# Ecogenomics/CheckM

Hardware: NVIDIA H100
Metric: genomes/hour (higher is better)
Workload: dtype int16 (SSV) / u8 (MSV) / int16 (Viterbi) / f32 (Forward, domain definition)

## Files before the change

checkm_b200/csrc/fwdback_blk.cuh:

```cuda
#pragma once
#include "device_utils.cuh"
#include "engine.hpp"
#include "fwdback.cuh"

namespace ckm {

constexpr int BLK_LOOKAHEAD_MAXQ = 16;

template <int Q, bool TSMEM>
struct BlkModel {
  int M;
  const float *rfb;
  const float4 *tsm;
  float4 t0[TSMEM ? 1 : Q], t1[TSMEM ? 1 : Q];
  int lane;
  __device__ __forceinline__ float4 T0(int q) const { return TSMEM ? tsm[q * 32 + lane] : t0[TSMEM ? 0 : q]; }
  __device__ __forceinline__ float4 T1(int q) const { return TSMEM ? tsm[(Q + q) * 32 + lane] : t1[TSMEM ? 0 : q]; }
};

template <int Q, bool TSMEM>
__device__ __forceinline__ void blk_model_load(BlkModel<Q, TSMEM> &bm, const ModelScalars &ms, const float4 *tfb, const float *rfb,
                                               float4 *tsm, int lane) {
  bm.M = ms.M; bm.lane = lane;
  bm.rfb = rfb + ms.blk_off * 32 * KPAD + lane;
  bm.tsm = tsm;
  const float4 *src = tfb + ms.blk_off * 32 * 2;
  if (TSMEM) {
    __syncwarp();
    for (int q = 0; q < Q; ++q) { tsm[q * 32 + lane] = __ldg(src + (q * 32 + lane) * 2); tsm[(Q + q) * 32 + lane] = __ldg(src + (q * 32 + lane) * 2 + 1); }
    __syncwarp();
  } else {
#pragma unroll
    for (int q = 0; q < Q; ++q) { bm.t0[TSMEM ? 0 : q] = __ldg(src + (q * 32 + lane) * 2); bm.t1[TSMEM ? 0 : q] = __ldg(src + (q * 32 + lane) * 2 + 1); }
  }
}

template <int Q, bool TSMEM, bool FULL, bool STORE_D = true>
__device__ __forceinline__ float forward_blk(const BlkModel<Q, TSMEM> &bm, const uint8_t *__restrict__ res, int L, const Specials sp,
                                             float *xmx, float *full) {
  const int lane = bm.lane;
  float Mx[Q], Ix[Q], Dx[Q];
#pragma unroll
  for (int q = 0; q < Q; ++q) { Mx[q] = 0.0f; Ix[q] = 0.0f; Dx[q] = 0.0f; }
  if (FULL) {
#pragma unroll
    for (int z = 0; z < 3 * Q; ++z) full[z * 32 + lane] = 0.0f;
  }
  float xE = 0.0f, xN = 1.0f, xJ = 0.0f, xB = sp.nmove, xC = 0.0f, totscale = 0.0f;
  if (xmx != nullptr && lane == 0) { xmx[X_E] = xE; xmx[X_N] = xN; xmx[X_J] = xJ; xmx[X_B] = xB; xmx[X_C] = xC; xmx[X_SCALE] = 1.0f; }
  constexpr bool LA = (Q <= BLK_LOOKAHEAD_MAXQ);
  float ecur[Q];
  int xnext;
  if (LA) {
    const float *rp = bm.rfb + (size_t)((L >= 1) ? __ldg(res) : 0) * Q * 32;
#pragma unroll
    for (int q = 0; q < Q; ++q) ecur[q] = __ldg(rp + q * 32);
    xnext = (L >= 2) ? __ldg(res + 1) : 0;
  } else xnext = (L >= 1) ? __ldg(res) : 0;
  for (int i = 1; i <= L; ++i) {
    float enext[LA ? Q : 1];
    {
      const float *rp = bm.rfb + (size_t)xnext * Q * 32;
      if (LA) {
#pragma unroll
        for (int q = 0; q < Q; ++q) enext[LA ? q : 0] = __ldg(rp + q * 32);
        xnext = (i + 2 <= L) ? __ldg(res + i + 1) : 0;
      } else {
#pragma unroll
        for (int q = 0; q < Q; ++q) ecur[q] = __ldg(rp + q * 32);
        xnext = (i + 1 <= L) ? __ldg(res + i) : 0;
      }
    }
    float pm_in = __shfl_up_sync(0xffffffffu, Mx[Q - 1], 1), pi_in = __shfl_up_sync(0xffffffffu, Ix[Q - 1], 1), pd_in = __shfl_up_sync(0xffffffffu, Dx[Q - 1], 1);
    if (lane == 0) { pm_in = 0.0f; pi_in = 0.0f; pd_in = 0.0f; }
    float md[Q], esum = 0.0f;
#pragma unroll
    for (int q = Q - 1; q >= 0; --q) {
      const float4 t0 = bm.T0(q), t1 = bm.T1(q);
      const float pm = (q > 0) ? Mx[q - 1] : pm_in, pi = (q > 0) ? Ix[q - 1] : pi_in, pd = (q > 0) ? Dx[q - 1] : pd_in;
      float sv = xB * t0.x;
      sv += pm * t0.y;
      sv += pi * t0.z;
      sv += pd * t0.w;
      sv *= ecur[q];
      const float nI = Mx[q] * t1.y + Ix[q] * t1.z;
      md[q] = sv * t1.x;
      Mx[q] = sv; Ix[q] = nI;
      esum += sv;
    }
    float Bb = 0.0f, Tb = 1.0f;
#pragma unroll
    for (int q = 0; q < Q; ++q) { const float tdd = bm.T1(q).w; Bb = md[q] + Bb * tdd; Tb *= tdd; }
    float Bs = Bb, Ts = Tb;
#pragma unroll
    for (int o = 1; o < 32; o <<= 1) {
      const float Bl = __shfl_up_sync(0xffffffffu, Bs, o), Tl = __shfl_up_sync(0xffffffffu, Ts, o);
      if (lane >= o) { Bs = Bs + Bl * Ts; Ts = Ts * Tl; }
    }
    float d = __shfl_up_sync(0xffffffffu, Bs, 1);
    if (lane == 0) d = 0.0f;
#pragma unroll
    for (int q = 0; q < Q; ++q) {
      const bool in = (lane * Q + q + 1) <= bm.M;
      Dx[q] = in ? d : 0.0f;
      esum += Dx[q];
      d = md[q] + d * bm.T1(q).w;
    }
    xE = warp_sum_float(esum);
    xN = xN * sp.nloop;
    xC = (xC * sp.nloop) + (xE * sp.emove);
    xJ = (xJ * sp.nloop) + (xE * sp.eloop);
    xB = (xJ * sp.nmove) + (xN * sp.nmove);
    float scale = 1.0f;
    if (xE > 1.0e4f) {
      scale = xE;
      const float inv = __fdiv_rn(1.0f, xE);
      xN = __fdiv_rn(xN, xE); xC = __fdiv_rn(xC, xE); xJ = __fdiv_rn(xJ, xE); xB = __fdiv_rn(xB, xE);
#pragma unroll
      for (int q = 0; q < Q; ++q) { Mx[q] *= inv; Dx[q] *= inv; Ix[q] *= inv; }
      totscale += (float)log((double)xE);
      xE = 1.0f;
    }
    if (FULL) {
      float *fr = full + (size_t)i * 3 * Q * 32 + lane;
#pragma unroll
      for (int q = 0; q < Q; ++q) { fr[q * 32] = Mx[q]; if (STORE_D) fr[(Q + q) * 32] = Dx[q]; fr[(2 * Q + q) * 32] = Ix[q]; }
    }
    if (xmx != nullptr && lane == 0) {
      float *xr = xmx + (size_t)i * X_NX;
      xr[X_E] = xE; xr[X_N] = xN; xr[X_J] = xJ; xr[X_B] = xB; xr[X_C] = xC; xr[X_SCALE] = scale;
    }
    if (LA) {
#pragma unroll
      for (int q = 0; q < Q; ++q) ecur[q] = enext[LA ? q : 0];
    }
  }
  return totscale + (float)log((double)(xC * sp.nmove));
}

__device__ __forceinline__ void prefetch_l2(const void *p) { asm volatile("prefetch.global.L2 [%0];" ::"l"(p)); }
template <int Q, bool TSMEM, int MODE>
__device__ __forceinline__ void backward_blk(const BlkModel<Q, TSMEM> &bm, const uint8_t *__restrict__ res, int L, const Specials sp,
                                             const float *fxmx, float *bxmx, float *full) {
  const int lane = bm.lane, M = bm.M;
  float Mx[Q], Ix[Q], Dx[Q];
#pragma unroll
  for (int q = 0; q < Q; ++q) { Mx[q] = 0.0f; Ix[q] = 0.0f; Dx[q] = 0.0f; }
  float xC = 0.0f, xE = 0.0f, xJ = 0.0f, xN = 0.0f, xB = 0.0f;
  constexpr bool LA = (Q <= BLK_LOOKAHEAD_MAXQ);
  float ecur[Q];
#pragma unroll
  for (int q = 0; q < Q; ++q) ecur[q] = 0.0f;
  int xnext = (L >= 1) ? __ldg(res + L - 1) : 0;
  for (int i = L; i >= 0; --i) {
    float enext[LA ? Q : 1];
    if (LA) {
      const float *rp = bm.rfb + (size_t)xnext * Q * 32;
#pragma unroll
      for (int q = 0; q < Q; ++q) enext[LA ? q : 0] = __ldg(rp + q * 32);
      xnext = (i >= 2) ? __ldg(res + i - 2) : 0;
    } else if (i < L) {
      const float *rp = bm.rfb + (size_t)xnext * Q * 32;
#pragma unroll
      for (int q = 0; q < Q; ++q) ecur[q] = __ldg(rp + q * 32);
      xnext = (i >= 1) ? __ldg(res + i - 1) : 0;
    }
    if (MODE == 2 && i >= 3) {
      const float *fr = full + (size_t)(i - 2) * 3 * Q * 32;
      if (lane < Q) { prefetch_l2(fr + lane * 32); prefetch_l2(fr + (2 * Q + lane) * 32); }
    }
    float em[Q];
    if (i == L) {
      xC = sp.nmove; xE = xC * sp.emove; xB = 0.0f; xJ = 0.0f; xN = 0.0f;
#pragma unroll
      for (int q = 0; q < Q; ++q) em[q] = 0.0f;
    } else {
      float part = 0.0f;
#pragma unroll
      for (int q = 0; q < Q; ++q) { em[q] = Mx[q] * ecur[q]; part += em[q] * bm.T0(q).x; }
      xB = warp_sum_float(part);
      xC = xC * sp.nloop;
      xJ = (xB * sp.nmove) + (xJ * sp.nloop);
      xN = (xB * sp.nmove) + (xN * sp.nloop);
      xE = (xC * sp.emove) + (xJ * sp.eloop);
    }
    const float s = (i >= 1) ? fxmx[(size_t)i * X_NX + X_SCALE] : 1.0f;
    if (i >= 1) {
      const float inv = (s > 1.0f) ? __fdiv_rn(1.0f, s) : 1.0f;
      float em_next = __shfl_down_sync(0xffffffffu, em[0], 1);
      float4 tn_next;
      {
        const float4 mine = bm.T0(0);
        tn_next.x = 0.0f;
        tn_next.y = __shfl_down_sync(0xffffffffu, mine.y, 1); tn_next.z = __shfl_down_sync(0xffffffffu, mine.z, 1); tn_next.w = __shfl_down_sync(0xffffffffu, mine.w, 1);
      }
      if (lane == 31) { em_next = 0.0f; tn_next.y = 0.0f; tn_next.z = 0.0f; tn_next.w = 0.0f; }
      float cb[Q];
      float Bb = 0.0f, Tb = 1.0f;
#pragma unroll
      for (int q = Q - 1; q >= 0; --q) {
        const int k = lane * Q + q + 1;
        const float mnext = (q < Q - 1) ? em[q + 1] : em_next;
        const float tdm = (q < Q - 1) ? bm.T0(q + 1).w : tn_next.w;
        const bool in = (k <= M);
        cb[q] = in ? (xE + ((k < M) ? mnext * tdm : 0.0f)) : 0.0f;
        const float tdd = in ? bm.T1(q).w : 0.0f;
        Bb = cb[q] + Bb * tdd; Tb *= tdd;
      }
      float Bs = Bb, Ts = Tb;
#pragma unroll
      for (int o = 1; o < 32; o <<= 1) {
        const float Br = __shfl_down_sync(0xffffffffu, Bs, o), Tr = __shfl_down_sync(0xffffffffu, Ts, o);
        if (lane + o < 32) { Bs = Bs + Br * Ts; Ts = Ts * Tr; }
      }
      float dnext = __shfl_down_sync(0xffffffffu, Bs, 1);
      if (lane == 31) dnext = 0.0f;
      float nM[Q], nI[Q], nD[Q];
#pragma unroll
      for (int q = Q - 1; q >= 0; --q) {
        const int k = lane * Q + q + 1;
        const bool in = (k <= M);
        const float4 t1 = bm.T1(q);
        const float mnext = (q < Q - 1) ? em[q + 1] : em_next;
        const float4 tn = (q < Q - 1) ? bm.T0(q + 1) : tn_next;
        const float tmm = (k < M) ? tn.y : 0.0f, tim = (k < M) ? tn.z : 0.0f;
        const float inext = (i < L) ? Ix[q] : 0.0f;
        const float dv = in ? (cb[q] + dnext * t1.w) : 0.0f;
        float mv = xE + mnext * tmm + inext * t1.y + dnext * t1.x;
        float iv = mnext * tim + inext * t1.z;
        if (!in) { mv = 0.0f; iv = 0.0f; }
        nM[q] = mv * inv; nI[q] = iv * inv; nD[q] = dv * inv;
        dnext = dv;
      }
#pragma unroll
      for (int q = 0; q < Q; ++q) { Mx[q] = nM[q]; Ix[q] = nI[q]; Dx[q] = nD[q]; }
      if (s > 1.0f) { xE = __fdiv_rn(xE, s); xN = __fdiv_rn(xN, s); xJ = __fdiv_rn(xJ, s); xB = __fdiv_rn(xB, s); xC = __fdiv_rn(xC, s); }
    } else {
      xC = 0.0f; xJ = 0.0f; xE = 0.0f;
#pragma unroll
      for (int q = 0; q < Q; ++q) { Mx[q] = 0.0f; Ix[q] = 0.0f; Dx[q] = 0.0f; }
    }
    if (MODE == 1) {
      float *fr = full + (size_t)i * 3 * Q * 32 + lane;
#pragma unroll
      for (int q = 0; q < Q; ++q) { fr[q * 32] = Mx[q]; fr[(Q + q) * 32] = Dx[q]; fr[(2 * Q + q) * 32] = Ix[q]; }
    }
    if (MODE == 2 && i >= 1) {
      float *fr = full + (size_t)i * 3 * Q * 32 + lane;
      float fm[Q], fi[Q];
#pragma unroll
      for (int q = 0; q < Q; ++q) { fm[q] = fr[q * 32]; fi[q] = fr[(2 * Q + q) * 32]; }
#pragma unroll
      for (int q = 0; q < Q; ++q) { fr[q * 32] = fm[q] * Mx[q]; fr[(2 * Q + q) * 32] = fi[q] * Ix[q]; }
    }
    if (bxmx != nullptr && lane == 0) {
      float *xr = bxmx + (size_t)i * X_NX;
      xr[X_E] = xE; xr[X_N] = xN; xr[X_J] = xJ; xr[X_B] = xB; xr[X_C] = xC; xr[X_SCALE] = s;
    }
    if (LA) {
#pragma unroll
      for (int q = 0; q < Q; ++q) ecur[q] = enext[LA ? q : 0];
    }
  }
}

}
```

checkm_b200/csrc/kernels_blk.cu:

```cuda
#include "engine.hpp"
#include "device_utils.cuh"
#include "stages.hpp"
#include "fwdback.cuh"
#include "fwdback_blk.cuh"
#include "domdef_common.cuh"
#include "filter_common.cuh"

namespace ckm {

constexpr int BLK_WARPS = 4;

__host__ __device__ constexpr size_t blk_tsm_bytes(int Q) { return (size_t)Q * 32 * 2 * sizeof(float4); }

template <int Q, bool TSMEM>
__global__ void __launch_bounds__(BLK_WARPS * 32) fwd2_kernel(FilterParams p) {
  extern __shared__ __align__(16) uint8_t bsm[];
  const int lane = threadIdx.x & 31, warp = threadIdx.x >> 5;
  float4 *tsm = reinterpret_cast<float4 *>(bsm) + (size_t)warp * Q * 32 * 2;
  const int n = min(*p.in_count, p.in_cap);
  for (int c = blockIdx.x * BLK_WARPS + warp; c < n; c += gridDim.x * BLK_WARPS) {
    Candidate cd = p.in[c];
    const ModelScalars ms = p.ms[cd.model];
    if (ms.vq != Q) continue;
    const int s = cd.seq, L = p.len[s];
    BlkModel<Q, TSMEM> bm;
    blk_model_load<Q, TSMEM>(bm, ms, p.tfb, p.rfb, tsm, lane);
    const float fsc = forward_blk<Q, TSMEM, false>(bm, p.res + p.off[s], L, make_specials(L, true), nullptr, nullptr);
    fwd_verdict(p, cd, fsc, ms, lane);
  }
}

template <int Q, bool TSMEM>
__global__ void __launch_bounds__(BLK_WARPS * 32) regions2_kernel(DomdefParams p) {
  extern __shared__ __align__(16) uint8_t bsm[];
  const int lane = threadIdx.x & 31, warp = threadIdx.x >> 5;
  float4 *tsm = reinterpret_cast<float4 *>(bsm) + (size_t)warp * Q * 32 * 2;
  for (int idx = p.pair_begin + blockIdx.x * BLK_WARPS + warp; idx < p.pair_end; idx += gridDim.x * BLK_WARPS) {
    const int pi = p.pair_order[idx];
    const PairWork pw = p.pairs[pi];
    const ModelScalars ms = p.ms[pw.model];
    if (ms.vq != Q) continue;
    const int L = pw.L;
    BlkModel<Q, TSMEM> bm;
    blk_model_load<Q, TSMEM>(bm, ms, p.tfb, p.rfb, tsm, lane);
    const uint8_t *res = p.res + p.off[pw.seq];
    const Specials sp = make_specials(L, true);
    float *xf = p.xf + pw.row_off * X_NX, *xb = p.xb + pw.row_off * X_NX;
    forward_blk<Q, TSMEM, false>(bm, res, L, sp, xf, nullptr);
    __syncwarp();
    backward_blk<Q, TSMEM, 0>(bm, res, L, sp, xf, xb, nullptr);
    __syncwarp();
    regions_tail(p, pi, L, sp, xf, xb, p.btot + pw.row_off, p.etot + pw.row_off, p.mocc + pw.row_off, p.n2sc + pw.row_off, lane);
    __syncwarp();
  }
}

template <int Q> struct BlockedLayout {
  const float *F; const float4 *tfb; int M;
  static __device__ __forceinline__ int at(int k) { return ((k - 1) % Q) * 32 + (k - 1) / Q; }
  __device__ __forceinline__ float cell(int row, int plane, int k) const { return F[((int64_t)row * 3 + plane) * (Q * 32) + at(k)]; }
  __device__ __forceinline__ float4 t0(int k) const { return __ldg(tfb + at(k) * 2); }
  __device__ __forceinline__ float4 t1(int k) const { return __ldg(tfb + at(k) * 2 + 1); }
  __device__ __forceinline__ void row_best(int row, int lane, float &bm, int &bk, float &bd, int &bdk) const {
    const float *dpc = F + (int64_t)row * 3 * (Q * 32) + lane;
    if constexpr (Q <= 12) {
#pragma unroll
      for (int q = 0; q < Q; ++q) {
        const int kk = lane * Q + q + 1;
        if (kk <= M) {
          const float v = dpc[q * 32]; if (v >= bm) { bm = v; bk = kk; }
          const float w = dpc[(Q + q) * 32]; if (w > bd) { bd = w; bdk = kk; }
        }
      }
    } else {
#pragma unroll 4
      for (int q = 0; q < Q; ++q) {
        const int kk = lane * Q + q + 1;
        if (kk <= M) { const float v = dpc[q * 32]; if (v >= bm) { bm = v; bk = kk; } }
      }
#pragma unroll 4
      for (int q = 0; q < Q; ++q) {
        const int kk = lane * Q + q + 1;
        if (kk <= M) { const float w = dpc[(Q + q) * 32]; if (w > bd) { bd = w; bdk = kk; } }
      }
    }
  }
};

template <int Q, bool TSMEM>
__global__ void __launch_bounds__(BLK_WARPS * 32) envelope2_kernel(DomdefParams p) {
  extern __shared__ __align__(16) uint8_t bsm[];
  const int lane = threadIdx.x & 31, warp = threadIdx.x >> 5;
  float4 *tsm = reinterpret_cast<float4 *>(bsm) + (size_t)warp * Q * 32 * 2;
  float *null2 = reinterpret_cast<float *>(bsm + (TSMEM ? BLK_WARPS * blk_tsm_bytes(Q) : 0)) + warp * 32;
  constexpr int QW = Q * 32;
  for (int idx = p.env_begin + blockIdx.x * BLK_WARPS + warp; idx < p.env_end; idx += gridDim.x * BLK_WARPS) {
    const int ei = p.env_order[idx];
    const Envelope env = p.envs[ei];
    const PairWork pw = p.pairs[env.pair];
    const ModelScalars ms = p.ms[pw.model];
    if (ms.vq != Q) continue;
    BlkModel<Q, TSMEM> bm;
    blk_model_load<Q, TSMEM>(bm, ms, p.tfb, p.rfb, tsm, lane);
    const int M = ms.M, Ld = env.j - env.i + 1;
    const uint8_t *res = p.res + p.off[pw.seq] + (env.i - 1);
    const Specials sp = make_specials(pw.L, false);
    const int64_t mat = (int64_t)(Ld + 1) * 3 * QW;
    float *F = p.scratch + env.scratch_off, *Bm = F;
    float *xf = F + mat, *xb = xf + (int64_t)(Ld + 1) * X_NX, *pps = xb + (int64_t)(Ld + 1) * X_NX;
    float *xo = xf;
    float *n2sc = p.n2sc + pw.row_off;
    const float envsc = forward_blk<Q, TSMEM, true, false>(bm, res, Ld, sp, xf, F);
    __syncwarp();
    backward_blk<Q, TSMEM, 2>(bm, res, Ld, sp, xf, xb, F);
    __syncwarp();
    const float scaleproduct = __fdiv_rn(1.0f, xb[X_N]);
    float em[Q], ein[Q];
#pragma unroll
    for (int q = 0; q < Q; ++q) { em[q] = 0.0f; ein[q] = 0.0f; }
    for (int r = 1; r <= Ld; ++r) {
      if (r + 2 <= Ld && lane < Q) {
        const float *fn = F + (int64_t)(r + 2) * 3 * QW;
        prefetch_l2(fn + lane * 32); prefetch_l2(fn + (2 * Q + lane) * 32);
      }
      const float totr = scaleproduct * xf[(int64_t)r * X_NX + X_SCALE];
      const float *fr = F + (int64_t)r * 3 * QW + lane;
      float vm[Q], vi[Q];
#pragma unroll
      for (int q = 0; q < Q; ++q) { vm[q] = fr[q * 32]; vi[q] = fr[(2 * Q + q) * 32]; }
#pragma unroll
      for (int q = 0; q < Q; ++q) {
        const float pm = vm[q] * totr, pi = vi[q] * totr;
        em[q] = (r == 1) ? pm : em[q] + pm;
        ein[q] = (r == 1) ? pi : ein[q] + pi;
      }
    }
    special_posteriors(sp, xf, xb, scaleproduct, pps, Ld, lane);
    const bool range_err = isinf(scaleproduct);
    if (!range_err && !env.null2_done) {
      const float norm = __fdiv_rn(1.0f, (float)Ld);
      const float xfactor = special_xfactor(pps, Ld, norm, lane);
#pragma unroll
      for (int q = 0; q < Q; ++q) { em[q] *= norm; ein[q] *= norm; }
      for (int x = 0; x < K; ++x) {
        const float *rp = bm.rfb + (size_t)x * QW;
        float part = 0.0f;
#pragma unroll
        for (int q = 0; q < Q; ++q) { part += em[q] * __ldg(rp + q * 32); part += ein[q]; }
        part = warp_sum_float(part);
        if (lane == 0) null2[x] = part + xfactor;
      }
      null2_finish(null2, n2sc, res, env, lane);
    }
    float oasc = 0.0f;
    const float NINF = -INFINITY;
    if (!range_err) {
      float oM[Q], oI[Q], oD[Q];
#pragma unroll
      for (int q = 0; q < Q; ++q) { oM[q] = NINF; oI[q] = NINF; oD[q] = NINF; }
#pragma unroll
      for (int z = 0; z < 3 * Q; ++z) Bm[z * 32 + lane] = NINF;
      OaSpecials os(sp);
      os.store(xo, lane);
      for (int r = 1; r <= Ld; ++r) {
        if (r + 2 <= Ld && lane < Q) {
          const float *fn = F + (int64_t)(r + 2) * 3 * QW;
          prefetch_l2(fn + lane * 32); prefetch_l2(fn + (2 * Q + lane) * 32);
        }
        const float totr = scaleproduct * xf[(int64_t)r * X_NX + X_SCALE];
        const float *ppr = F + (int64_t)r * 3 * QW + lane;
        float *orow = Bm + (int64_t)r * 3 * QW + lane;
        float ppm[Q], ppi[Q];
#pragma unroll
        for (int q = 0; q < Q; ++q) { ppm[q] = ppr[q * 32]; ppi[q] = ppr[(2 * Q + q) * 32]; }
        float pm_in = __shfl_up_sync(0xffffffffu, oM[Q - 1], 1), pi_in = __shfl_up_sync(0xffffffffu, oI[Q - 1], 1), pd_in = __shfl_up_sync(0xffffffffu, oD[Q - 1], 1);
        if (lane == 0) { pm_in = NINF; pi_in = NINF; pd_in = NINF; }
        float a[Q]; bool ps[Q];
        float emax = NINF;
#pragma unroll
        for (int q = Q - 1; q >= 0; --q) {
          const float4 t0 = bm.T0(q), t1 = bm.T1(q);
          const bool in = (lane * Q + q + 1) <= M;
          const float pm = (q > 0) ? oM[q - 1] : pm_in, pi = (q > 0) ? oI[q - 1] : pi_in, pd = (q > 0) ? oD[q - 1] : pd_in;
          float sv = (t0.x > 0.0f) ? os.B : 0.0f;
          sv = fmaxf(sv, (t0.y > 0.0f) ? pm : 0.0f);
          sv = fmaxf(sv, (t0.z > 0.0f) ? pi : 0.0f);
          sv = fmaxf(sv, (t0.w > 0.0f) ? pd : 0.0f);
          sv += ppm[q] * totr;
          if (!in) sv = NINF;
          const float nI = in ? fmaxf((t1.y > 0.0f) ? oM[q] : 0.0f, (t1.z > 0.0f) ? oI[q] : 0.0f) + ppi[q] * totr : NINF;
          a[q] = (t1.x > 0.0f) ? sv : 0.0f;
          ps[q] = (t1.w > 0.0f);
          if (!in) { a[q] = NINF; ps[q] = true; }
          if (!ps[q]) a[q] = fmaxf(a[q], 0.0f);
          oM[q] = sv; oI[q] = nI;
          emax = fmaxf(emax, sv);
        }
        float A = NINF; bool pass = true;
#pragma unroll
        for (int q = 0; q < Q; ++q) { if (ps[q]) { A = fmaxf(a[q], A); } else { A = a[q]; pass = false; } }
        float As = A; bool Ps = pass;
#pragma unroll
        for (int o = 1; o < 32; o <<= 1) {
          const float Al = __shfl_up_sync(0xffffffffu, As, o);
          const int pl = __shfl_up_sync(0xffffffffu, (int)Ps, o);
          if (lane >= o && Ps) { As = fmaxf(As, Al); Ps = (pl != 0); }
        }
        float d = __shfl_up_sync(0xffffffffu, As, 1);
        if (lane == 0) d = NINF;
#pragma unroll
        for (int q = 0; q < Q; ++q) {
          const bool in = (lane * Q + q + 1) <= M;
          oD[q] = in ? d : NINF;
          emax = fmaxf(emax, oD[q]);
          d = ps[q] ? fmaxf(a[q], d) : a[q];
        }
#pragma unroll
        for (int o = 16; o > 0; o >>= 1) emax = fmaxf(emax, __shfl_xor_sync(0xffffffffu, emax, o));
        os.row(sp, pps + r * 3, emax);
#pragma unroll
        for (int q = 0; q < Q; ++q) { orow[q * 32] = oM[q]; orow[(Q + q) * 32] = oD[q]; orow[(2 * Q + q) * 32] = oI[q]; }
        os.store(xo + (int64_t)r * X_NX, lane);
      }
      oasc = os.C;
    }
    __syncwarp();
    OaTrace tr;
    if (!range_err) tr = oa_traceback(BlockedLayout<Q>{Bm, p.tfb + ms.blk_off * 64, M}, p, pw, env, sp, xo, pps, Ld, M, lane);
    write_domain(p, env, n2sc, tr, envsc, oasc, lane);
    __syncwarp();
  }
}

template <class P, class KF>
static int launch_blk(KF kern, const char *name, int Q, bool tsmem, const P &p, int grid, size_t extra, cudaStream_t st) {
  return launch_kernel(kern, name, grid, BLK_WARPS * 32, (tsmem ? BLK_WARPS * blk_tsm_bytes(Q) : 0) + extra, st, p);
}
int launch_fwd2(const FilterParams &p, int cls, int grid, cudaStream_t st) {
  return with_class(cls, [&](auto Q, auto TSMEM) { return launch_blk(fwd2_kernel<Q, TSMEM>, "fwd2_kernel", Q, TSMEM, p, grid, 0, st); });
}
int launch_regions2(const DomdefParams &p, int cls, int grid, cudaStream_t st) {
  return with_class(cls, [&](auto Q, auto TSMEM) { return launch_blk(regions2_kernel<Q, TSMEM>, "regions2_kernel", Q, TSMEM, p, grid, 0, st); });
}
int launch_envelopes2(const DomdefParams &p, int cls, int grid, cudaStream_t st) {
  return with_class(cls, [&](auto Q, auto TSMEM) {
    return launch_blk(envelope2_kernel<Q, TSMEM>, "envelope2_kernel", Q, TSMEM, p, grid, BLK_WARPS * 32 * sizeof(float), st);
  });
}

}
```

Before: 35540.

## Recompute forward rows in envelope OA pass instead of storing full matrix

For small Q the envelope kernel no longer stores the full forward DP matrix. Backward writes its M/I rows, and the optimal-accuracy pass recomputes each forward row on the fly to form posteriors. The null2 posterior sums are folded into that same pass, with the accumulators kept in shared memory for some Q, and launch bounds gain minimum-block hints. This trades extra forward arithmetic for much less global-memory traffic to the scratch matrix, but it risks register pressure and occupancy changes.

```diff
diff --git a/checkm_b200/csrc/fwdback_blk.cuh b/checkm_b200/csrc/fwdback_blk.cuh
--- a/checkm_b200/csrc/fwdback_blk.cuh
+++ b/checkm_b200/csrc/fwdback_blk.cuh
@@ -35,29 +35,26 @@
   }
 }
 
-template <int Q, bool TSMEM, bool FULL, bool STORE_D = true>
-__device__ __forceinline__ float forward_blk(const BlkModel<Q, TSMEM> &bm, const uint8_t *__restrict__ res, int L, const Specials sp,
-                                             float *xmx, float *full) {
-  const int lane = bm.lane;
+template <int Q, bool TSMEM>
+struct FwdRows {
+  static constexpr bool LA = (Q <= BLK_LOOKAHEAD_MAXQ);
   float Mx[Q], Ix[Q], Dx[Q];
-#pragma unroll
-  for (int q = 0; q < Q; ++q) { Mx[q] = 0.0f; Ix[q] = 0.0f; Dx[q] = 0.0f; }
-  if (FULL) {
-#pragma unroll
-    for (int z = 0; z < 3 * Q; ++z) full[z * 32 + lane] = 0.0f;
-  }
-  float xE = 0.0f, xN = 1.0f, xJ = 0.0f, xB = sp.nmove, xC = 0.0f, totscale = 0.0f;
-  if (xmx != nullptr && lane == 0) { xmx[X_E] = xE; xmx[X_N] = xN; xmx[X_J] = xJ; xmx[X_B] = xB; xmx[X_C] = xC; xmx[X_SCALE] = 1.0f; }
-  constexpr bool LA = (Q <= BLK_LOOKAHEAD_MAXQ);
+  float xE, xN, xJ, xB, xC, totscale;
   float ecur[Q];
   int xnext;
-  if (LA) {
-    const float *rp = bm.rfb + (size_t)((L >= 1) ? __ldg(res) : 0) * Q * 32;
-#pragma unroll
-    for (int q = 0; q < Q; ++q) ecur[q] = __ldg(rp + q * 32);
-    xnext = (L >= 2) ? __ldg(res + 1) : 0;
-  } else xnext = (L >= 1) ? __ldg(res) : 0;
-  for (int i = 1; i <= L; ++i) {
+  __device__ __forceinline__ void init(const BlkModel<Q, TSMEM> &bm, const uint8_t *__restrict__ res, int L, const Specials &sp) {
+#pragma unroll
+    for (int q = 0; q < Q; ++q) { Mx[q] = 0.0f; Ix[q] = 0.0f; Dx[q] = 0.0f; }
+    xE = 0.0f; xN = 1.0f; xJ = 0.0f; xB = sp.nmove; xC = 0.0f; totscale = 0.0f;
+    if (LA) {
+      const float *rp = bm.rfb + (size_t)((L >= 1) ? __ldg(res) : 0) * Q * 32;
+#pragma unroll
+      for (int q = 0; q < Q; ++q) ecur[q] = __ldg(rp + q * 32);
+      xnext = (L >= 2) ? __ldg(res + 1) : 0;
+    } else xnext = (L >= 1) ? __ldg(res) : 0;
+  }
+  __device__ __forceinline__ float row(const BlkModel<Q, TSMEM> &bm, const uint8_t *__restrict__ res, int L, const Specials &sp, int i) {
+    const int lane = bm.lane;
     float enext[LA ? Q : 1];
     {
       const float *rp = bm.rfb + (size_t)xnext * Q * 32;
@@ -121,21 +118,39 @@
       totscale += (float)log((double)xE);
       xE = 1.0f;
     }
+    if (LA) {
+#pragma unroll
+      for (int q = 0; q < Q; ++q) ecur[q] = enext[LA ? q : 0];
+    }
+    return scale;
+  }
+  __device__ __forceinline__ float score(const Specials &sp) const { return totscale + (float)log((double)(xC * sp.nmove)); }
+};
+
+template <int Q, bool TSMEM, bool FULL = false, bool STORE_D = true>
+__device__ __forceinline__ float forward_blk(const BlkModel<Q, TSMEM> &bm, const uint8_t *__restrict__ res, int L, const Specials sp,
+                                             float *xmx, float *full = nullptr) {
+  const int lane = bm.lane;
+  FwdRows<Q, TSMEM> f;
+  f.init(bm, res, L, sp);
+  if (FULL) {
+#pragma unroll
+    for (int z = 0; z < 3 * Q; ++z) full[z * 32 + lane] = 0.0f;
+  }
+  if (xmx != nullptr && lane == 0) { xmx[X_E] = f.xE; xmx[X_N] = f.xN; xmx[X_J] = f.xJ; xmx[X_B] = f.xB; xmx[X_C] = f.xC; xmx[X_SCALE] = 1.0f; }
+  for (int i = 1; i <= L; ++i) {
+    const float scale = f.row(bm, res, L, sp, i);
     if (FULL) {
       float *fr = full + (size_t)i * 3 * Q * 32 + lane;
 #pragma unroll
-      for (int q = 0; q < Q; ++q) { fr[q * 32] = Mx[q]; if (STORE_D) fr[(Q + q) * 32] = Dx[q]; fr[(2 * Q + q) * 32] = Ix[q]; }
+      for (int q = 0; q < Q; ++q) { fr[q * 32] = f.Mx[q]; if (STORE_D) fr[(Q + q) * 32] = f.Dx[q]; fr[(2 * Q + q) * 32] = f.Ix[q]; }
     }
     if (xmx != nullptr && lane == 0) {
       float *xr = xmx + (size_t)i * X_NX;
-      xr[X_E] = xE; xr[X_N] = xN; xr[X_J] = xJ; xr[X_B] = xB; xr[X_C] = xC; xr[X_SCALE] = scale;
-    }
-    if (LA) {
-#pragma unroll
-      for (int q = 0; q < Q; ++q) ecur[q] = enext[LA ? q : 0];
-    }
-  }
-  return totscale + (float)log((double)(xC * sp.nmove));
+      xr[X_E] = f.xE; xr[X_N] = f.xN; xr[X_J] = f.xJ; xr[X_B] = f.xB; xr[X_C] = f.xC; xr[X_SCALE] = scale;
+    }
+  }
+  return f.score(sp);
 }
 
 __device__ __forceinline__ void prefetch_l2(const void *p) { asm volatile("prefetch.global.L2 [%0];" ::"l"(p)); }
@@ -240,10 +255,10 @@
 #pragma unroll
       for (int q = 0; q < Q; ++q) { Mx[q] = 0.0f; Ix[q] = 0.0f; Dx[q] = 0.0f; }
     }
-    if (MODE == 1) {
+    if (MODE == 1 && i >= 1) {
       float *fr = full + (size_t)i * 3 * Q * 32 + lane;
 #pragma unroll
-      for (int q = 0; q < Q; ++q) { fr[q * 32] = Mx[q]; fr[(Q + q) * 32] = Dx[q]; fr[(2 * Q + q) * 32] = Ix[q]; }
+      for (int q = 0; q < Q; ++q) { fr[q * 32] = Mx[q]; fr[(2 * Q + q) * 32] = Ix[q]; }
     }
     if (MODE == 2 && i >= 1) {
       float *fr = full + (size_t)i * 3 * Q * 32 + lane;
diff --git a/checkm_b200/csrc/kernels_blk.cu b/checkm_b200/csrc/kernels_blk.cu
--- a/checkm_b200/csrc/kernels_blk.cu
+++ b/checkm_b200/csrc/kernels_blk.cu
@@ -25,7 +25,7 @@
     const int s = cd.seq, L = p.len[s];
     BlkModel<Q, TSMEM> bm;
     blk_model_load<Q, TSMEM>(bm, ms, p.tfb, p.rfb, tsm, lane);
-    const float fsc = forward_blk<Q, TSMEM, false>(bm, p.res + p.off[s], L, make_specials(L, true), nullptr, nullptr);
+    const float fsc = forward_blk<Q, TSMEM>(bm, p.res + p.off[s], L, make_specials(L, true), nullptr);
     fwd_verdict(p, cd, fsc, ms, lane);
   }
 }
@@ -46,7 +46,7 @@
     const uint8_t *res = p.res + p.off[pw.seq];
     const Specials sp = make_specials(L, true);
     float *xf = p.xf + pw.row_off * X_NX, *xb = p.xb + pw.row_off * X_NX;
-    forward_blk<Q, TSMEM, false>(bm, res, L, sp, xf, nullptr);
+    forward_blk<Q, TSMEM>(bm, res, L, sp, xf);
     __syncwarp();
     backward_blk<Q, TSMEM, 0>(bm, res, L, sp, xf, xb, nullptr);
     __syncwarp();
@@ -87,12 +87,27 @@
   }
 };
 
+__host__ __device__ constexpr bool env_recompute(int Q) { return Q <= 16; }
+__host__ __device__ constexpr bool env_sums_smem(int Q) { return Q == 16 || Q == 20 || Q == 32; }
+__host__ __device__ constexpr size_t env_sums_bytes(int Q) { return env_sums_smem(Q) ? (size_t)2 * Q * 32 * sizeof(float) : 0; }
+__host__ __device__ constexpr int env_min_blocks(int Q) { return Q <= 2 ? 4 : Q <= 6 ? 3 : 1; }
+
+template <int Q, bool SMEM>
+struct EnvSums {
+  float rm[SMEM ? 1 : Q], ri[SMEM ? 1 : Q];
+  float *s; int lane;
+  __device__ __forceinline__ float &m(int q) { return SMEM ? s[q * 32 + lane] : rm[SMEM ? 0 : q]; }
+  __device__ __forceinline__ float &i(int q) { return SMEM ? s[(Q + q) * 32 + lane] : ri[SMEM ? 0 : q]; }
+};
+
 template <int Q, bool TSMEM>
-__global__ void __launch_bounds__(BLK_WARPS * 32) envelope2_kernel(DomdefParams p) {
+__global__ void __launch_bounds__(BLK_WARPS * 32, env_min_blocks(Q)) envelope2_kernel(DomdefParams p) {
   extern __shared__ __align__(16) uint8_t bsm[];
   const int lane = threadIdx.x & 31, warp = threadIdx.x >> 5;
   float4 *tsm = reinterpret_cast<float4 *>(bsm) + (size_t)warp * Q * 32 * 2;
-  float *null2 = reinterpret_cast<float *>(bsm + (TSMEM ? BLK_WARPS * blk_tsm_bytes(Q) : 0)) + warp * 32;
+  uint8_t *wsm = bsm + (TSMEM ? BLK_WARPS * blk_tsm_bytes(Q) : 0);
+  float *sums = reinterpret_cast<float *>(wsm) + (size_t)warp * 2 * Q * 32;
+  float *null2 = reinterpret_cast<float *>(wsm + BLK_WARPS * env_sums_bytes(Q)) + warp * 32;
   constexpr int QW = Q * 32;
   for (int idx = p.env_begin + blockIdx.x * BLK_WARPS + warp; idx < p.env_end; idx += gridDim.x * BLK_WARPS) {
     const int ei = p.env_order[idx];
@@ -106,73 +121,55 @@
     const uint8_t *res = p.res + p.off[pw.seq] + (env.i - 1);
     const Specials sp = make_specials(pw.L, false);
     const int64_t mat = (int64_t)(Ld + 1) * 3 * QW;
-    float *F = p.scratch + env.scratch_off, *Bm = F;
-    float *xf = F + mat, *xb = xf + (int64_t)(Ld + 1) * X_NX, *pps = xb + (int64_t)(Ld + 1) * X_NX;
+    float *Bm = p.scratch + env.scratch_off;
+    float *xf = Bm + mat, *xb = xf + (int64_t)(Ld + 1) * X_NX, *pps = xb + (int64_t)(Ld + 1) * X_NX;
     float *xo = xf;
     float *n2sc = p.n2sc + pw.row_off;
-    const float envsc = forward_blk<Q, TSMEM, true, false>(bm, res, Ld, sp, xf, F);
-    __syncwarp();
-    backward_blk<Q, TSMEM, 2>(bm, res, Ld, sp, xf, xb, F);
+    constexpr bool RECOMPUTE = env_recompute(Q);
+    const float envsc = forward_blk<Q, TSMEM, !RECOMPUTE, false>(bm, res, Ld, sp, xf, RECOMPUTE ? nullptr : Bm);
+    __syncwarp();
+    backward_blk<Q, TSMEM, RECOMPUTE ? 1 : 2>(bm, res, Ld, sp, xf, xb, Bm);
     __syncwarp();
     const float scaleproduct = __fdiv_rn(1.0f, xb[X_N]);
-    float em[Q], ein[Q];
-#pragma unroll
-    for (int q = 0; q < Q; ++q) { em[q] = 0.0f; ein[q] = 0.0f; }
-    for (int r = 1; r <= Ld; ++r) {
-      if (r + 2 <= Ld && lane < Q) {
-        const float *fn = F + (int64_t)(r + 2) * 3 * QW;
-        prefetch_l2(fn + lane * 32); prefetch_l2(fn + (2 * Q + lane) * 32);
-      }
-      const float totr = scaleproduct * xf[(int64_t)r * X_NX + X_SCALE];
-      const float *fr = F + (int64_t)r * 3 * QW + lane;
-      float vm[Q], vi[Q];
-#pragma unroll
-      for (int q = 0; q < Q; ++q) { vm[q] = fr[q * 32]; vi[q] = fr[(2 * Q + q) * 32]; }
-#pragma unroll
-      for (int q = 0; q < Q; ++q) {
-        const float pm = vm[q] * totr, pi = vi[q] * totr;
-        em[q] = (r == 1) ? pm : em[q] + pm;
-        ein[q] = (r == 1) ? pi : ein[q] + pi;
-      }
-    }
     special_posteriors(sp, xf, xb, scaleproduct, pps, Ld, lane);
     const bool range_err = isinf(scaleproduct);
-    if (!range_err && !env.null2_done) {
-      const float norm = __fdiv_rn(1.0f, (float)Ld);
-      const float xfactor = special_xfactor(pps, Ld, norm, lane);
-#pragma unroll
-      for (int q = 0; q < Q; ++q) { em[q] *= norm; ein[q] *= norm; }
-      for (int x = 0; x < K; ++x) {
-        const float *rp = bm.rfb + (size_t)x * QW;
-        float part = 0.0f;
-#pragma unroll
-        for (int q = 0; q < Q; ++q) { part += em[q] * __ldg(rp + q * 32); part += ein[q]; }
-        part = warp_sum_float(part);
-        if (lane == 0) null2[x] = part + xfactor;
-      }
-      null2_finish(null2, n2sc, res, env, lane);
-    }
     float oasc = 0.0f;
     const float NINF = -INFINITY;
     if (!range_err) {
+      EnvSums<Q, env_sums_smem(Q)> n2;
+      n2.s = sums; n2.lane = lane;
       float oM[Q], oI[Q], oD[Q];
 #pragma unroll
-      for (int q = 0; q < Q; ++q) { oM[q] = NINF; oI[q] = NINF; oD[q] = NINF; }
+      for (int q = 0; q < Q; ++q) { n2.m(q) = 0.0f; n2.i(q) = 0.0f; oM[q] = NINF; oI[q] = NINF; oD[q] = NINF; }
 #pragma unroll
       for (int z = 0; z < 3 * Q; ++z) Bm[z * 32 + lane] = NINF;
       OaSpecials os(sp);
       os.store(xo, lane);
+      FwdRows<Q, TSMEM> f;
+      if (RECOMPUTE) f.init(bm, res, Ld, sp);
       for (int r = 1; r <= Ld; ++r) {
         if (r + 2 <= Ld && lane < Q) {
-          const float *fn = F + (int64_t)(r + 2) * 3 * QW;
-          prefetch_l2(fn + lane * 32); prefetch_l2(fn + (2 * Q + lane) * 32);
-        }
-        const float totr = scaleproduct * xf[(int64_t)r * X_NX + X_SCALE];
-        const float *ppr = F + (int64_t)r * 3 * QW + lane;
+          const float *bn = Bm + (int64_t)(r + 2) * 3 * QW;
+          prefetch_l2(bn + lane * 32); prefetch_l2(bn + (2 * Q + lane) * 32);
+        }
         float *orow = Bm + (int64_t)r * 3 * QW + lane;
         float ppm[Q], ppi[Q];
-#pragma unroll
-        for (int q = 0; q < Q; ++q) { ppm[q] = ppr[q * 32]; ppi[q] = ppr[(2 * Q + q) * 32]; }
+        if constexpr (RECOMPUTE) {
+          const float totr = scaleproduct * f.row(bm, res, Ld, sp, r);
+#pragma unroll
+          for (int q = 0; q < Q; ++q) { ppm[q] = (f.Mx[q] * orow[q * 32]) * totr; ppi[q] = (f.Ix[q] * orow[(2 * Q + q) * 32]) * totr; }
+        } else {
+          const float totr = scaleproduct * xf[(int64_t)r * X_NX + X_SCALE];
+#pragma unroll
+          for (int q = 0; q < Q; ++q) { ppm[q] = orow[q * 32]; ppi[q] = orow[(2 * Q + q) * 32]; }
+#pragma unroll
+          for (int q = 0; q < Q; ++q) { ppm[q] = ppm[q] * totr; ppi[q] = ppi[q] * totr; }
+        }
+#pragma unroll
+        for (int q = 0; q < Q; ++q) {
+          n2.m(q) = (r == 1) ? ppm[q] : n2.m(q) + ppm[q];
+          n2.i(q) = (r == 1) ? ppi[q] : n2.i(q) + ppi[q];
+        }
         float pm_in = __shfl_up_sync(0xffffffffu, oM[Q - 1], 1), pi_in = __shfl_up_sync(0xffffffffu, oI[Q - 1], 1), pd_in = __shfl_up_sync(0xffffffffu, oD[Q - 1], 1);
         if (lane == 0) { pm_in = NINF; pi_in = NINF; pd_in = NINF; }
         float a[Q]; bool ps[Q];
@@ -186,9 +183,9 @@
           sv = fmaxf(sv, (t0.y > 0.0f) ? pm : 0.0f);
           sv = fmaxf(sv, (t0.z > 0.0f) ? pi : 0.0f);
           sv = fmaxf(sv, (t0.w > 0.0f) ? pd : 0.0f);
-          sv += ppm[q] * totr;
+          sv += ppm[q];
           if (!in) sv = NINF;
-          const float nI = in ? fmaxf((t1.y > 0.0f) ? oM[q] : 0.0f, (t1.z > 0.0f) ? oI[q] : 0.0f) + ppi[q] * totr : NINF;
+          const float nI = in ? fmaxf((t1.y > 0.0f) ? oM[q] : 0.0f, (t1.z > 0.0f) ? oI[q] : 0.0f) + ppi[q] : NINF;
           a[q] = (t1.x > 0.0f) ? sv : 0.0f;
           ps[q] = (t1.w > 0.0f);
           if (!in) { a[q] = NINF; ps[q] = true; }
@@ -223,6 +220,21 @@
         os.store(xo + (int64_t)r * X_NX, lane);
       }
       oasc = os.C;
+      if (!env.null2_done) {
+        const float norm = __fdiv_rn(1.0f, (float)Ld);
+        const float xfactor = special_xfactor(pps, Ld, norm, lane);
+#pragma unroll
+        for (int q = 0; q < Q; ++q) { n2.m(q) *= norm; n2.i(q) *= norm; }
+        for (int x = 0; x < K; ++x) {
+          const float *rp = bm.rfb + (size_t)x * QW;
+          float part = 0.0f;
+#pragma unroll
+          for (int q = 0; q < Q; ++q) { part += n2.m(q) * __ldg(rp + q * 32); part += n2.i(q); }
+          part = warp_sum_float(part);
+          if (lane == 0) null2[x] = part + xfactor;
+        }
+        null2_finish(null2, n2sc, res, env, lane);
+      }
     }
     __syncwarp();
     OaTrace tr;
@@ -244,7 +256,7 @@
 }
 int launch_envelopes2(const DomdefParams &p, int cls, int grid, cudaStream_t st) {
   return with_class(cls, [&](auto Q, auto TSMEM) {
-    return launch_blk(envelope2_kernel<Q, TSMEM>, "envelope2_kernel", Q, TSMEM, p, grid, BLK_WARPS * 32 * sizeof(float), st);
+    return launch_blk(envelope2_kernel<Q, TSMEM>, "envelope2_kernel", Q, TSMEM, p, grid, BLK_WARPS * (env_sums_bytes(Q) + 32 * sizeof(float)), st);
   });
 }
 
```

After: 36190, median of 6. +1.8%, better.
